# tiborcamargo/KinectPy

Hardware: AMD Instinct MI355X
Metric: Mpoints/sec end-to-end (unproject+filter+ICP), 4-sensor frame (higher is better)
Workload: dtype f64 decisions / f32 storage

## Files before the change

### kinectpy_amd/csrc/kpx_icp.hip

```cpp
#include <chrono>
#include <mutex>
#include <fcntl.h>
#include <memory>
#include <condition_variable>
#include <thread>
#include <atomic>
#include <sys/file.h>
#include <unistd.h>
#include <limits.h>
#include <stddef.h>
#include <string.h>
#include <stdio.h>
#include <time.h>
#include <stdlib.h>

#include "kpx_internal.h"
#include "kpx_linalg.h"
#include "kpx_fixed.h"

namespace kpx {

typedef double d4 __attribute__((ext_vector_type(4)));
#ifndef KPX_ICP_ACQ_FENCE
#define KPX_ICP_ACQ_FENCE 1
// ... 1023 lines not shown
    uint32_t my_cert = 0u;
    const bool certs = fuse.ticket && fuse.light_key && fuse.cert;
    if (PERSIST && k > 0) {
        if (lane < 16) {
            my_row = rowi[wave][lane][1];
#pragma unroll
            for (int a = 0; a < 3; ++a) { my_src[a] = rowsrc[wave][lane][a]; my_pt[a] = rowk[wave][lane][a]; my_nrm[a] = rowk[wave][lane][3 + a]; }
            my_prev = __float_as_int(rowk[wave][lane][6]);
            if (certs) my_cert = rowc[wave][lane];
        }
    } else if (lane < 16) {
        const int64_t r = row_base + lane < last ? row_base + lane : last;
        if (idx_cur || d2_cur) my_row = row_of[r];
#pragma unroll
        for (int a = 0; a < 3; ++a) my_src[a] = src_sorted[3 * r + a];
        if (PERSIST) {
#pragma unroll
            for (int a = 0; a < 3; ++a) rowsrc[wave][lane][a] = my_src[a];
            rowc[wave][lane] = 0u;
        }
        if (k > 0) {
            my_prev = idx_sorted[r];
#pragma unroll
            for (int a = 0; a < 3; ++a) my_pt[a] = ptgt_sorted[3 * r + a];
            if (certs) my_cert = fuse.cert[r];
        }
    }
    __shared__ double s_thist[kCertHist][12];
    if (PERSIST) {
        if (certs && k < kCertHist && tix < 12) s_thist[k][tix] = st->T[tix];
    } else if (certs && k > 0)
        for (int e = tix; e < 12 * (k < kCertHist ? k : kCertHist); e += kIThreads) (&s_thist[0][0])[e] = fuse.thist[e];
    GroupPre gpre;
    group_pre_load(gpre, group_box, n_groups, lane);
    if (!PERSIST && mode == 1 && k > 0 && lane < 16) {
        const float *np_ = tn + 3 * (int64_t)(my_prev > 0 ? my_prev : 0);
#pragma unroll
        for (int a = 0; a < 3; ++a) my_nrm[a] = np_[a];
    }
    const double *Tk = st->T;
    static_assert(sizeof(IcpState) % sizeof(double) == 0, "IcpState is copied as doubles");
    if (KPX_ICP_STATE_LDS && fuse.ticket && tix < sizeof(IcpState) / sizeof(double))
        reinterpret_cast<double *>(&s_state)[tix] = reinterpret_cast<const double *>(st)[tix];
    if (fuse.pair) {
        const IcpState *in = fuse.pair + ((k + 1) & 1);
        IcpState *out = fuse.pair + (k & 1);
        const unsigned long long *prev = fuse.ring + (int64_t)((k + 2) % 3) * kAccSet;
        if (k > 0 && tix < kAcc) s_sums[tix] = (int)tix < (mode == 1 ? kAcc : 17) ? fixed_total(prev, tix) : 0.0;
        if (tix == 0) s_state = *in;
        __syncthreads();
        if (s_state.done) {
            if (bid == 0 && tix == 0) *out = s_state;
            return;
        }
        __shared__ FinishScratch s_fs;
        if (k > 0 && wave == 0)
            icp_finish_wave(s_sums, n, mode, k - 1, fuse.max_iter, fuse.rel_fit, fuse.rel_rmse, &s_state, bid == 0 ? fuse.result : (double *)nullptr,
                            s_fs, lane);
        __syncthreads();
        if (bid == 0) {
            unsigned long long *next = fuse.ring + (int64_t)((k + 1) % 3) * kAccSet;
            for (int e = tix; e < kAccSet; e += kIThreads) next[e] = 0ull;
            if (tix == 0) {
                *out = s_state;
                if (k > 0 && fuse.progress)
                    __hip_atomic_store(fuse.progress, fuse.tag | ((unsigned long long)(s_state.done ? 1 : 0) << 32) | (unsigned long long)(unsigned)k,
                                       __ATOMIC_RELEASE, __HIP_MEMORY_SCOPE_SYSTEM);
            }
        }
        if (s_state.done) return;
        Tk = s_state.T;
        acc = fuse.ring + (int64_t)(k % 3) * kAccSet;
    } else if (st->done) return;
    bool skip = false;
    if (fuse.ticket && fuse.light_key) {
        const double key = PERSIST ? (k > 0 ? s_key : 0.0) : fuse.light_key[bid];
        skip = key > 0.0 && (st->motion + st->reach) * (1.0 + 1e-6) + 1e-6 < key;
    }
    __shared__ double s_light[kIWaves];
    const int nacc = mode == 1 ? kAcc : 17;
    if (tile_visits && tix == 0 && bid < kStampBlocks) { g_icp_stamp[bid][7] = skip ? 1ull : 0ull; g_icp_stamp[bid][6] = (unsigned long long)nblocks; }
    do {
    if (skip) break;
    __shared__ int32_t lists[kIWaves][kLScratch];
    __shared__ double rowd[kIWaves][16][kRowStride];
    __shared__ float rowf[kIWaves][16][kRowFStride];
    __shared__ double sh[kAcc][kIRows + 1];
    if (tile_visits && tix == 0 && bid < kStampBlocks) {
        g_icp_stamp[bid][0] = t_block_start;
        g_icp_stamp[bid][6] = (unsigned long long)nblocks;
    }
    phase_tick(tile_visits, 1, bid);
    if (certs && (k > 0 || PERSIST)) __syncthreads();
    if (PERSIST && fuse.stamp && tix == 0) {
        const unsigned long long t = wall_clock64();
        if (bid == 0) fuse.stamp[0] = t;
        atomicMax(&fuse.stamp[5], t);
        atomicMin(&fuse.stamp[10], t);
    }

    const double c_reach = certs ? st->reach : 0.0;
    double c_skin = 0.0;
    if (certs && k > 0) {
        const double lm = st->last_motion, md = sqrt(max_d2);
        if (lm <= (double)fuse.pol.calm * md) c_skin = fmin(fmax((double)fuse.pol.factor * lm, (double)fuse.pol.smin * md), (double)fuse.pol.smax * md);
    }
    bool my_active = true, my_certd = false;
    if (lane < 16) {
        const int64_t i = my_row;
        double s[3];
        xform_row(Tk, my_src, s);
        const double seed = row_seed(s);
        double bv = INFINITY;
        int32_t bj = INT_MAX;
        if (k > 0) {
            const int32_t p = my_prev;
            if (p >= 0) {
                const double tx = my_pt[0], ty = my_pt[1], tz = my_pt[2];
                const double t2 = fma(tx, tx, fma(ty, ty, tz * tz));
                double d = fma(s[0], -2.0 * tx, seed);
                d = fma(s[1], -2.0 * ty, d);
                d = fma(s[2], -2.0 * tz, d);
                bv = fma(1.0, t2, d);
                bj = p;
            }
        }
        const double clamp = (max_d2 + 1.0) * (1.0 + 9.31322574615478515625e-10) + ldexp(seed + t2max + 1.0, -38);
        if (!(bv <= clamp)) { bv = clamp; bj = INT_MAX; }
        double rb0 = bv - 1.0;
        if (certs) {
            double d1 = c_reach;
            if (bj != INT_MAX) {
                const double dx = s[0] - (double)my_pt[0], dy = s[1] - (double)my_pt[1], dz = s[2] - (double)my_pt[2];
                d1 = sqrt(fma(dz, dz, fma(dy, dy, dx * dx))) * (1.0 + 1e-12);
            }
            const bool keeps = (my_prev >= 0) == (bj != INT_MAX);
            const int kc = (int)(my_cert & 63u);
            const float Lc = __uint_as_float(my_cert & ~63u);
            double pc[3] = { 0.0, 0.0, 0.0 };
            if (Lc > 0.0f) {
                const double *Th = s_thist[kc];
                const double x = my_src[0], y = my_src[1], z = my_src[2];
#pragma unroll
                for (int a = 0; a < 3; ++a) pc[a] = fma(Th[4 * a], x, fma(Th[4 * a + 1], y, fma(Th[4 * a + 2], z, Th[4 * a + 3])));
            }
            const double ex = s[0] - pc[0], ey = s[1] - pc[1], ez = s[2] - pc[2];
            const double moved = sqrt(fma(ez, ez, fma(ey, ey, ex * ex))) * (1.0 + 1e-12);
            const bool certd = Lc > 0.0f && keeps && (d1 + moved) * (1.0 + 1e-6) + 1e-6 < (double)Lc;
            my_active = (!certd || fuse.cert_check) && row_base + lane <= last;
            my_certd = certd && row_base + lane <= last;
            if (certd && !fuse.cert_check) rb0 = -1.0;
            else if (c_skin > 0.0) { const double rr = d1 + c_skin; rb0 = fmax(rb0, rr * rr); }
        }
        rowd[wave][lane][0] = s[0]; rowd[wave][lane][1] = s[1]; rowd[wave][lane][2] = s[2];
        rowd[wave][lane][3] = rb0;
        rowd[wave][lane][4] = seed; rowd[wave][lane][5] = bv;
        rowi[wave][lane][0] = bj; rowi[wave][lane][1] = (int32_t)i;
#pragma unroll
        for (int a = 0; a < 3; ++a) { rowk[wave][lane][a] = my_pt[a]; rowk[wave][lane][3 + a] = my_nrm[a]; }
        rowk[wave][lane][6] = __int_as_float(my_prev);
    }
    if (PERSIST && fuse.stamp) {
        const bool searched = lane < 16 && my_active && !my_certd;
        const unsigned long long sm = __builtin_amdgcn_ballot_w64(searched);
        const unsigned long long np = __builtin_amdgcn_ballot_w64(searched && my_prev < 0);
        const unsigned long long nc = __builtin_amdgcn_ballot_w64(searched && (my_cert & ~63u) == 0u);
        if (lane == 0 && sm) {
            atomicAdd(&fuse.stamp[26], 1ull); atomicAdd(&fuse.stamp[27], (unsigned long long)__builtin_popcountll(sm));
            atomicAdd(&fuse.stamp[28], (unsigned long long)__builtin_popcountll(np)); atomicAdd(&fuse.stamp[29], (unsigned long long)__builtin_popcountll(nc));
        }
// ... 12 lines not shown
        w.best[r] = rowd[wave][rr][5];
        w.bcol[r] = rowi[wave][rr][0];
        w.rb0[r] = rowd[wave][rr][3];
    }
    w.skin = c_skin;
    w.act_mask = act_mask;
    w.light_gap2 = -1.0;
    w.dbg = (PERSIST && fuse.stamp && bid == 0 && wave == 0) ? fuse.stamp + 16 : (unsigned long long *)nullptr;
    phase_tick(tile_visits, 2, bid);
    if (PERSIST) chain_tick(fuse.stamp, 1, bid == 0 && tix == 0);
    const unsigned long long t_sweep = tile_visits ? wall_clock64() : 0ull;
    unsigned long long swept = 0ull;
    int lane_p = 0, wave_p = 0, q_p = 0, j_p = 0;
    int64_t row_base_p = 0;
    auto rederive = [&]() {
        lane_p = opaque_i((int)(threadIdx.x & 63)); wave_p = opaque_i((int)(threadIdx.x >> 6)); q_p = lane_p >> 4; j_p = lane_p & 15;
        row_base_p = ((int64_t)bid * kIWaves + wave_p) * kLRows;
    };
    if (act_mask != 0u) {
        wave_lds_fence();
        swept = sweep_wave<true, true, PERSIST>(w, Bs, orig, tile_box, group_box, n_groups, t2max, lists[wave], &gpre);
        rederive();
        if (certs && fuse.cert_check && j_p == 0) {
#pragma unroll
            for (int r = 0; r < 4; ++r) {
                const int rr = q_p + 4 * r;
                if (((certd_mask >> rr) & 1u) != 0u && w.bcol[r] != rowi[wave_p][rr][0]) {
                    if (atomicAdd(&g_cert_check[2], 1ull) == 0ull) {
                        g_cert_check[3] = (unsigned long long)k; g_cert_check[4] = (unsigned long long)(row_base_p + rr);
                        g_cert_check[5] = (unsigned long long)(unsigned)rowi[wave_p][rr][0]; g_cert_check[6] = (unsigned long long)(unsigned)w.bcol[r];
                        g_cert_check[7] = (unsigned long long)((PERSIST ? rowc[wave_p][rr] : fuse.cert[row_base_p + rr]) & ~63u);
                    }
                }
            }
        }
        if (certs && j_p == 0) {
#pragma unroll
            for (int r = 0; r < 4; ++r) {
                const int rr = q_p + 4 * r;
                if (((act_mask >> rr) & 1u) != 0u && ((certd_mask >> rr) & 1u) == 0u) {
                    typedef unsigned uu2 __attribute__((ext_vector_type(2)));
                    const uu2 pat = { 0u, w.sec[r] };
                    const double d2nd = w.sec[r] == 0xFFFFFFFFu ? INFINITY : __builtin_bit_cast(double, pat) - 1.0 - w.eps_out;
                    const double l2 = fmin(w.rb_out[r], d2nd);
                    const uint32_t lb = l2 > 0.0 && k < kCertHist ? (__float_as_uint(f32_down(sqrt(l2) * (1.0 - 1e-7))) & ~63u) : 0u;
                    const uint32_t cw = lb > 63u ? (lb | (uint32_t)k) : 0u;
                    if (PERSIST) rowc[wave_p][rr] = cw; else fuse.cert[row_base_p + rr] = cw;
                }
            }
        }
    }
    if (act_mask == 0u) rederive();
    __shared__ int s_cnt[kIWaves];
    if (lane_p == 0) s_cnt[wave_p] = __builtin_popcount(act_mask & ~certd_mask);
    const unsigned visited = (unsigned)(swept & 0xFFFFu);
    if (certs && fuse.cert_check && lane_p == 0) {
        if (bid == 0 && wave_p == 0 && g_cert_check[2] == 0ull) {
            g_cert_check[3] = (unsigned long long)k; g_cert_check[4] = __builtin_bit_cast(unsigned long long, st->last_motion);
            g_cert_check[5] = __builtin_bit_cast(unsigned long long, st->motion); g_cert_check[6] = __builtin_bit_cast(unsigned long long, c_skin);
        }
        atomicAdd(&g_cert_check[0], (unsigned long long)__builtin_popcount(certd_mask));
        atomicAdd(&g_cert_check[1], (unsigned long long)__builtin_popcount(act_mask & ~certd_mask));
    }
    if (lane_p == 0) s_light[wave_p] = act_mask == 0xFFFFu ? w.light_gap2 : -1.0;
    if (tile_visits && lane_p == 0 && bid < kStampBlocks && kIWaves <= 4) {
        unsigned long long *o = g_icp_wave[bid * 4 + wave_p];
        int with = 0;
#pragma unroll
        for (int r = 0; r < 4; ++r) with += (w.bcol[r] >= 0 && w.bcol[r] != INT_MAX) ? 1 : 0;
        o[0] = t_sweep; o[1] = wall_clock64(); o[2] = swept; o[3] = (unsigned long long)with;
    }
    phase_tick(tile_visits, 3, bid);
    if (PERSIST) chain_tick(fuse.stamp, 2, bid == 0 && lane_p == 0 && wave_p == 0);
    if (PERSIST && fuse.stamp && bid == 0 && lane_p == 0 && wave_p == 0) { fuse.stamp[13] = swept; fuse.stamp[14] = (unsigned long long)act_mask | ((unsigned long long)certd_mask << 16); }
    if (tile_visits && lane_p == 0) atomicAdd(tile_visits + ((bid * kIWaves + wave_p) & (kVisitSlots - 1)), (unsigned long long)visited);
    wave_lds_fence();
    if (j_p == 0) {
#pragma unroll
        for (int r = 0; r < 4; ++r) rowi[wave_p][q_p + 4 * r][0] = w.bcol[r];
    }
    wave_lds_fence();

    const int lane_e = lane_p, wave_e = wave_p;
    if (lane_e < 16) {
        const int col = wave_e * 16 + lane_e;
        for (int a = 0; a < nacc; ++a) sh[a][col] = 0.0;
        if (row_base_p + lane_e <= last) {
            const int32_t bj = rowi[wave_e][lane_e][0];
            const int64_t i = rowi[wave_e][lane_e][1];
            const bool none = bj < 0 || bj == INT_MAX;
            const int32_t out_j = none ? -1 : bj;
            const int32_t prev_j = __float_as_int(rowk[wave_e][lane_e][6]);
            const bool changed = k == 0 || out_j != prev_j;
            if (idx_cur) idx_cur[i] = out_j;
            if (PERSIST) rowk[wave_e][lane_e][6] = __int_as_float(out_j);
            else if (changed) idx_sorted[row_base_p + lane_e] = out_j;
            if (none) {
                if (d2_cur) d2_cur[i] = INFINITY;
            } else {
                const double s[3] = { rowd[wave_e][lane_e][0], rowd[wave_e][lane_e][1], rowd[wave_e][lane_e][2] };
                float tf[3] = { rowk[wave_e][lane_e][0], rowk[wave_e][lane_e][1], rowk[wave_e][lane_e][2] }, nf[3] = { rowk[wave_e][lane_e][3], rowk[wave_e][lane_e][4], rowk[wave_e][lane_e][5] };
                if (changed) {
                    const float *tp = tgt + 3 * (int64_t)bj;
#pragma unroll
                    for (int c = 0; c < 3; ++c) tf[c] = tp[c];
                    if (mode == 1) {
                        const float *np_ = tn + 3 * (int64_t)bj;
#pragma unroll
                        for (int c = 0; c < 3; ++c) nf[c] = np_[c];
                    }
#pragma unroll
                    for (int c = 0; c < 3; ++c) {
                        if (PERSIST) { rowk[wave_e][lane_e][c] = tf[c]; rowk[wave_e][lane_e][3 + c] = nf[c]; }
                        else ptgt_sorted[3 * (row_base_p + lane_e) + c] = tf[c];
                    }
                }
                const double t[3] = { (double)tf[0], (double)tf[1], (double)tf[2] };
                const double dx = s[0] - t[0], dy = s[1] - t[1], dz = s[2] - t[2];
                const double d2 = fma(dz, dz, fma(dy, dy, dx * dx));
                if (d2_cur) d2_cur[i] = d2;
                if (d2 < max_d2) {
                    sh[0][col] = 1.0; sh[1][col] = d2;
#pragma unroll
                    for (int c = 0; c < 3; ++c) { sh[2 + c][col] = s[c]; sh[5 + c][col] = t[c]; }
#pragma unroll
                    for (int a = 0; a < 3; ++a)
#pragma unroll
                        for (int c = 0; c < 3; ++c) sh[8 + 3 * a + c][col] = t[a] * s[c];
                    if (mode == 1) {
                        const double nx = nf[0], ny = nf[1], nz = nf[2];
                        const double res = (s[0] - t[0]) * nx + (s[1] - t[1]) * ny + (s[2] - t[2]) * nz;
                        const double J[6] = { s[1] * nz - s[2] * ny, s[2] * nx - s[0] * nz, s[0] * ny - s[1] * nx, nx, ny, nz };
                        int slot = 17;
#pragma unroll
                        for (int a = 0; a < 6; ++a)
#pragma unroll
                            for (int c = a; c < 6; ++c) sh[slot++][col] = J[a] * J[c];
#pragma unroll
                        for (int a = 0; a < 6; ++a) sh[38 + a][col] = J[a] * res;
                    }
                }
            }
        }
    }
    __syncthreads();
    phase_tick(tile_visits, 4, bid);
    const int tix_e = wave_e * 64 + lane_e;
    if (tix_e < nacc) {
        unsigned long long lo = 0ull, hi = 0ull;
#pragma unroll
        for (int t = 0; t < kIWaves; ++t) {
            unsigned long long l, h;
            fixed_split(tile_tree16(&sh[tix_e][16 * t]), l, h);
            fixed_accumulate(lo, hi, l, h);
        }
        unsigned long long *slot = acc + (((int64_t)(bid & (kAccCopies - 1)) * kAcc + tix_e) * kFixedWords);
        if (fuse.ticket) fixed_add_words_performed(slot, lo, hi); else fixed_add_words(slot, lo, hi);
    } else if (!PERSIST && fuse.ticket && tix_e == nacc) {
        int cnt = 0;
#pragma unroll
        for (int wv = 0; wv < kIWaves; ++wv) cnt += s_cnt[wv];
        if (cnt) {
            const unsigned long long back = __hip_atomic_fetch_add(fuse.ticket + kSearchedWord + (bid & 7u), (unsigned long long)cnt, __ATOMIC_RELAXED, __HIP_MEMORY_SCOPE_AGENT);
            asm volatile("" ::"v"(back));
        }
    }
    if (fuse.light_key && tix == kIThreads - 1) {
        double g2 = INFINITY;
        bool light = true;
#pragma unroll
        for (int wv = 0; wv < kIWaves; ++wv) { light = light && s_light[wv] >= 0.0; g2 = fmin(g2, s_light[wv]); }
        const double nk = light ? st->motion + sqrt(g2) * (1.0 - 1e-9) : 0.0;
        if (PERSIST) s_key = nk; else fuse.light_key[bid] = nk;
    }
    phase_tick(tile_visits, 5, bid);
    } while (false);
    if (PERSIST && fuse.stamp && tix == 0) {
        const unsigned long long t = wall_clock64();
        if (bid == 0) fuse.stamp[3] = t;
        atomicMax(&fuse.stamp[11], t);
    }
    if (!fuse.ticket) return;
    __shared__ unsigned s_ticket;
    __syncthreads();
    if (tix == 0) s_ticket = (unsigned)__hip_atomic_fetch_add(fuse.ticket, 1ull, __ATOMIC_RELAXED, __HIP_MEMORY_SCOPE_AGENT);
    __syncthreads();
    if (PERSIST && fuse.stamp && tix == 0) {
        const unsigned long long t = wall_clock64();
        if (bid == 0) fuse.stamp[4] = t;
        atomicMax(&fuse.stamp[6], t);
    }
    if (s_ticket != nblocks - 1u) return;
#if KPX_ICP_ACQ_FENCE
    __builtin_amdgcn_fence(__ATOMIC_ACQUIRE, "agent");
#endif
    const int tix_w = opaque_i((int)threadIdx.x);
    if (tix_w < kAcc) s_sums[tix_w] = tix_w < nacc ? fixed_total_coherent(acc, tix_w) : 0.0;
    const unsigned long long n_searched = PERSIST ? 0ull : searched_take(fuse.ticket, tix_w);
    __syncthreads();
    if (PERSIST) chain_tick(fuse.stamp, 7, tix == 0);
    for (int e = tix_w; e < kAccSet; e += kIThreads) __hip_atomic_store(acc + e, 0ull, __ATOMIC_RELAXED, __HIP_MEMORY_SCOPE_AGENT);
    if (tix == 0) __hip_atomic_store(fuse.ticket, 0ull, __ATOMIC_RELAXED, __HIP_MEMORY_SCOPE_AGENT);
    if (PERSIST) asm volatile("s_waitcnt vmcnt(0)" ::: "memory");
    if (wave != 0) {
        if (PERSIST) __syncthreads();
        return;
    }
    __shared__ FinishScratch s_tail;
    const double *tbbox_w = tbbox;
    asm volatile("" : "+s"(tbbox_w));
    const double t2max_w = target_t2max(tbbox_w);
    IcpState *stw = const_cast<IcpState *>(st);
    IcpState *work = KPX_ICP_STATE_LDS ? &s_state : stw;
    if (PERSIST)
        icp_finish_wave_call(s_sums, n, mode, k, fuse.max_iter, fuse.rel_fit, fuse.rel_rmse, work, (double *)nullptr, &s_tail, lane,
                             fuse.light_key ? fuse.sbbox : (const double *)nullptr, max_d2, t2max_w, fuse.stamp ? fuse.stamp + 32 : (unsigned long long *)nullptr);
    else
        icp_finish_wave(s_sums, n, mode, k, fuse.max_iter, fuse.rel_fit, fuse.rel_rmse, work, fuse.result, s_tail, lane,
                        LightSkip{ fuse.light_key ? fuse.sbbox : (const double *)nullptr, max_d2, t2max_w });
    wave_lds_fence();
    if (PERSIST) chain_tick(fuse.stamp, 8, lane == 0);
    if (PERSIST) {
        static_assert(KPX_ICP_STATE_LDS, "the chain form updates the LDS copy of the state");
        static_assert(sizeof(IcpState) == kChainWords * sizeof(double), "record layout");
        __syncthreads();
        if (lane < kChainWords)
            __hip_atomic_store(reinterpret_cast<unsigned long long *>(fuse.chain_rec + (size_t)kChainRec * (k + 1)) + lane,
                               reinterpret_cast<const unsigned long long *>(&s_state)[lane], __ATOMIC_RELAXED, __HIP_MEMORY_SCOPE_AGENT);
        if (work->done && fuse.result) {
            if (lane < 16) fuse.result[lane] = work->T[lane];
            if (lane == 0) { fuse.result[16] = work->fitness; fuse.result[17] = work->rmse; fuse.result[18] = (double)k; fuse.result[19] = work->count; }
        }
        if (lane == 0 && fuse.progress && work->done)
            __hip_atomic_store(fuse.progress, fuse.tag | (1ull << 32) | (unsigned long long)(unsigned)(k + 1), __ATOMIC_RELAXED, __HIP_MEMORY_SCOPE_SYSTEM);
        chain_tick(fuse.stamp, 9, lane == 0);
        if (fuse.stamp && lane == 0) fuse.stamp[12] = __builtin_amdgcn_s_memtime();
// ... 1532 lines not shown
```

### kinectpy_amd/csrc/kpx_icprows.h

```cpp
#pragma once

namespace kpx {

constexpr int kRowsBatchMax = 16;
constexpr int kRowsBlock = 64;
struct RowsProblem {
    const float *src_sorted;
    int32_t *idx_sorted;
    float *ptgt_sorted;
    uint32_t *cert;
    double *thist;
    double *light_key;
    const double *sbbox;
    IcpState *state;
    unsigned long long *ring;
    double *result;
    unsigned long long *progress;
    unsigned long long tag;
    const float *tgt, *tn;
    const double *Bs;
    const int32_t *orig;
    const float *tile_box, *group_box;
    const double *tbbox;
    int64_t n;
    int32_t n_groups, k;
    uint32_t block0, blocks;
};
struct RowsArgs {
    RowsProblem p[kRowsBatchMax];
    int32_t count;
};

constexpr int kDppXor1 = 0xB1, kDppXor2 = 0x4E, kDppHalfMirror = 0x141, kDppMirror = 0x140;
__device__ __forceinline__ double row16_tree_sum(double v)
{
    v += dpp_f64<kDppXor1>(v);
    v += dpp_f64<kDppXor2>(v);
    v += dpp_f64<kDppHalfMirror>(v);
    v += dpp_f64<kDppMirror>(v);
    return v;
}

template <int MODE, int R>
__global__ __launch_bounds__(64) __attribute__((amdgpu_waves_per_eu(KPX_ICP_WPE, KPX_ICP_WPE))) void icp_rows_kernel(RowsArgs args, double max_d2, int max_iter, double rel_fit,
                                                                                                                     double rel_rmse, unsigned long long *__restrict__ tile_visits,
                                                                                                                     int light, CertPolicy pol)
{
    constexpr int NACC = MODE == 1 ? kAcc : 17;
    static_assert(R == 16 || R == 32 || R == 64, "rows per wave");
    int pi = 0;
#pragma unroll
    for (int c = 1; c < kRowsBatchMax; ++c) pi += (c < args.count && blockIdx.x >= args.p[c].block0) ? 1 : 0;
    const RowsProblem &P = args.p[pi];
    const unsigned bid = blockIdx.x - P.block0;
    const int k = P.k;
    IcpState *const st = P.state;
    if (st->done) return;

    __shared__ IcpState s_state;
    __shared__ double s_sums[kAcc];
    __shared__ FinishScratch s_tail;
    __shared__ double rowd[kRowsBlock][kRowStride];
    __shared__ float rowf[kLRows][kRowFStride];
    __shared__ float rowk[kRowsBlock][11];
    __shared__ int32_t rowi[kRowsBlock];
    __shared__ uint32_t rowc[kRowsBlock];
    __shared__ int32_t rowm[kRowsBlock];
    __shared__ int32_t lists[kLScratch];
    static_assert(kLScratch * sizeof(int32_t) >= 4 * kAcc * sizeof(double), "the tile partials reuse the sweep's scratch");
    double (*s_part)[kAcc] = reinterpret_cast<double (*)[kAcc]>(lists);

    const int lane = threadIdx.x;
    const unsigned long long lt = (1ull << lane) - 1ull;
    const int64_t last = P.n - 1;
    const int64_t row = (int64_t)bid * R + lane;
    const bool valid = lane < R && row <= last;
    const int64_t r = valid ? row : last;
    const bool certs = (light & 2) != 0, use_light = (light & 1) != 0, cert_check = (light & 4) != 0;
    const double t2max = target_t2max(P.tbbox);

    float my_src[3], my_pt[3] = { 0.0f, 0.0f, 0.0f }, my_nrm[3] = { 0.0f, 0.0f, 0.0f };
    int32_t my_prev = -1;
    uint32_t my_cert = 0u;
#pragma unroll
    for (int a = 0; a < 3; ++a) my_src[a] = P.src_sorted[3 * r + a];
    if (k > 0) {
        my_prev = P.idx_sorted[r];
#pragma unroll
        for (int a = 0; a < 3; ++a) my_pt[a] = P.ptgt_sorted[3 * r + a];
        if (certs) my_cert = P.cert[r];
    }
    const double key_in = use_light ? P.light_key[bid] : 0.0;
    if (lane < (int)(sizeof(IcpState) / sizeof(double))) reinterpret_cast<double *>(&s_state)[lane] = reinterpret_cast<const double *>(st)[lane];
    GroupPre gpre;
    group_pre_load(gpre, P.group_box, P.n_groups, lane);
    if (MODE == 1 && k > 0) {
        const float *np_ = P.tn + 3 * (int64_t)(my_prev > 0 ? my_prev : 0);
#pragma unroll
        for (int a = 0; a < 3; ++a) my_nrm[a] = np_[a];
    }
    double Th[12];
    const int kc = (int)(my_cert & 63u);
    const float Lc = __uint_as_float(my_cert & ~63u);
    if (certs && k > 0 && Lc > 0.0f) {
#pragma unroll
        for (int e = 0; e < 12; ++e) Th[e] = P.thist[12 * kc + e];
    } else {
#pragma unroll
        for (int e = 0; e < 12; ++e) Th[e] = 0.0;
    }
    const double *Tk = st->T;
    unsigned long long *const ticket = P.ring + kAccSet;

    const bool skip = use_light && key_in > 0.0 && (st->motion + st->reach) * (1.0 + 1e-6) + 1e-6 < key_in;
    unsigned visited_total = 0u;
    if (!skip) {
        const double c_reach = certs ? st->reach : 0.0;
        double c_skin = 0.0;
        if (certs && k > 0) {
            const double lm = st->last_motion, md = sqrt(max_d2);
            if (lm <= (double)pol.calm * md) c_skin = fmin(fmax((double)pol.factor * lm, (double)pol.smin * md), (double)pol.smax * md);
        }
        bool my_active = valid, my_certd = false;
        unsigned long long act64, certd64;
        int n_act;
        {
            double s[3];
            xform_row(Tk, my_src, s);
            const double seed = row_seed(s);
            double bv = INFINITY;
            int32_t bj = INT_MAX;
            if (k > 0 && my_prev >= 0) {
                const double tx = my_pt[0], ty = my_pt[1], tz = my_pt[2];
                const double t2 = fma(tx, tx, fma(ty, ty, tz * tz));
                double d = fma(s[0], -2.0 * tx, seed);
                d = fma(s[1], -2.0 * ty, d);
                d = fma(s[2], -2.0 * tz, d);
                bv = fma(1.0, t2, d);
                bj = my_prev;
            }
            const double clamp = (max_d2 + 1.0) * (1.0 + 9.31322574615478515625e-10) + ldexp(seed + t2max + 1.0, -38);
            if (!(bv <= clamp)) { bv = clamp; bj = INT_MAX; }
            double rb0 = bv - 1.0;
            if (certs) {
                double d1 = c_reach;
                if (bj != INT_MAX) {
                    const double dx = s[0] - (double)my_pt[0], dy = s[1] - (double)my_pt[1], dz = s[2] - (double)my_pt[2];
                    d1 = sqrt(fma(dz, dz, fma(dy, dy, dx * dx))) * (1.0 + 1e-12);
                }
                const bool keeps = (my_prev >= 0) == (bj != INT_MAX);
                double pc[3] = { 0.0, 0.0, 0.0 };
                if (Lc > 0.0f) {
                    const double x = my_src[0], y = my_src[1], z = my_src[2];
#pragma unroll
                    for (int a = 0; a < 3; ++a) pc[a] = fma(Th[4 * a], x, fma(Th[4 * a + 1], y, fma(Th[4 * a + 2], z, Th[4 * a + 3])));
                }
                const double ex = s[0] - pc[0], ey = s[1] - pc[1], ez = s[2] - pc[2];
                const double moved = sqrt(fma(ez, ez, fma(ey, ey, ex * ex))) * (1.0 + 1e-12);
                const bool certd = Lc > 0.0f && keeps && (d1 + moved) * (1.0 + 1e-6) + 1e-6 < (double)Lc;
                my_active = (!certd || cert_check) && valid;
                my_certd = certd && valid;
                if (certd && !cert_check) rb0 = -1.0;
                else if (c_skin > 0.0) { const double rr = d1 + c_skin; rb0 = fmax(rb0, rr * rr); }
            }
            act64 = __builtin_amdgcn_ballot_w64(my_active);
            certd64 = __builtin_amdgcn_ballot_w64(my_certd);
            n_act = __builtin_popcountll(act64);
            if (my_active) {
                const int slot = __builtin_popcountll(act64 & lt);
                rowd[slot][0] = s[0]; rowd[slot][1] = s[1]; rowd[slot][2] = s[2];
                rowd[slot][3] = rb0;
                rowd[slot][4] = seed; rowd[slot][5] = bv;
                rowi[slot] = bj;
                rowc[slot] = my_cert;
                rowm[slot] = my_certd ? 1 : 0;
            }
            if (lane >= n_act) {
                rowd[lane][0] = 0.0; rowd[lane][1] = 0.0; rowd[lane][2] = 0.0;
                rowd[lane][3] = -1.0;
                rowd[lane][4] = 1.0; rowd[lane][5] = 2.0;
                rowi[lane] = INT_MAX;
                rowc[lane] = 0u;
                rowm[lane] = 1;
            }
#pragma unroll
            for (int a = 0; a < 3; ++a) { rowk[lane][a] = my_pt[a]; rowk[lane][3 + a] = my_nrm[a]; rowk[lane][7 + a] = my_src[a]; }
            rowk[lane][6] = __int_as_float(my_prev);
        }
        wave_lds_fence();

        bool light_blk = n_act == R;
        double gap2_blk = INFINITY;
#pragma unroll 1
        for (int v0 = 0; v0 < n_act; v0 += kLRows) {
            const int left = n_act - v0;
            const unsigned act_mask = left >= kLRows ? 0xFFFFu : ((1u << left) - 1u);
            const int lane_s = opaque_i((int)threadIdx.x), q_s = lane_s >> 4, j_s = lane_s & 15;
            WaveRows w;
            w.rows = &rowd[v0][0];
            w.rowsf = &rowf[0][0];
            w.a = q_s < 3 ? rowd[v0 + j_s][q_s] : 1.0;
#pragma unroll
            for (int rr4 = 0; rr4 < 4; ++rr4) {
                const int rr = v0 + q_s + 4 * rr4;
                w.seed[rr4] = rowd[rr][4];
                w.best[rr4] = rowd[rr][5];
                w.bcol[rr4] = rowi[rr];
                w.rb0[rr4] = rowd[rr][3];
            }
            w.skin = c_skin;
            w.act_mask = act_mask;
            w.light_gap2 = -1.0;
            w.dbg = nullptr;
            wave_lds_fence();
            const unsigned long long swept = sweep_wave<true, true, true>(w, P.Bs, P.orig, P.tile_box, P.group_box, P.n_groups, t2max, lists, &gpre);
            visited_total += (unsigned)(swept & 0xFFFFu);
            const int lane_p = opaque_i((int)threadIdx.x), q_p = lane_p >> 4, j_p = lane_p & 15;
            if (certs && cert_check && j_p == 0) {
#pragma unroll
                for (int rr4 = 0; rr4 < 4; ++rr4) {
                    const int rr = q_p + 4 * rr4;
                    if (((act_mask >> rr) & 1u) != 0u && rowm[v0 + rr] != 0 && w.bcol[rr4] != rowi[v0 + rr]) {
                        if (atomicAdd(&g_cert_check[2], 1ull) == 0ull) {
                            g_cert_check[3] = (unsigned long long)k; g_cert_check[4] = (unsigned long long)((int64_t)bid * R + v0 + rr);
                            g_cert_check[5] = (unsigned long long)(unsigned)rowi[v0 + rr]; g_cert_check[6] = (unsigned long long)(unsigned)w.bcol[rr4];
                            g_cert_check[7] = (unsigned long long)(rowc[v0 + rr] & ~63u);
                        }
                    }
                }
            }
            wave_lds_fence();
            if (j_p == 0) {
#pragma unroll
                for (int rr4 = 0; rr4 < 4; ++rr4) {
                    const int rr = q_p + 4 * rr4;
                    rowi[v0 + rr] = w.bcol[rr4];
                    if (certs && ((act_mask >> rr) & 1u) != 0u && rowm[v0 + rr] == 0) {
                        typedef unsigned uu2 __attribute__((ext_vector_type(2)));
                        const uu2 pat = { 0u, w.sec[rr4] };
                        const double d2nd = w.sec[rr4] == 0xFFFFFFFFu ? INFINITY : __builtin_bit_cast(double, pat) - 1.0 - w.eps_out;
                        const double l2 = fmin(w.rb_out[rr4], d2nd);
                        const uint32_t lb = l2 > 0.0 && k < kCertHist ? (__float_as_uint(f32_down(sqrt(l2) * (1.0 - 1e-7))) & ~63u) : 0u;
                        rowc[v0 + rr] = lb > 63u ? (lb | (uint32_t)k) : 0u;
                    }
                }
            }
            if (w.light_gap2 >= 0.0) gap2_blk = fmin(gap2_blk, w.light_gap2);
            else light_blk = false;
            wave_lds_fence();
        }
        const int lane_e = opaque_i((int)threadIdx.x);
        const unsigned long long lt_e = (1ull << lane_e) - 1ull;
        if (certs && cert_check && lane_e == 0) {
            if (bid == 0 && g_cert_check[2] == 0ull) {
                g_cert_check[3] = (unsigned long long)k; g_cert_check[4] = __builtin_bit_cast(unsigned long long, st->last_motion);
                g_cert_check[5] = __builtin_bit_cast(unsigned long long, st->motion); g_cert_check[6] = __builtin_bit_cast(unsigned long long, c_skin);
            }
            atomicAdd(&g_cert_check[0], (unsigned long long)__builtin_popcountll(certd64));
            atomicAdd(&g_cert_check[1], (unsigned long long)__builtin_popcountll(act64 & ~certd64));
        }
        if (tile_visits && lane_e == 0 && visited_total) atomicAdd(tile_visits + (blockIdx.x & (kVisitSlots - 1)), (unsigned long long)visited_total);

        double c[NACC];
#pragma unroll
        for (int a = 0; a < NACC; ++a) c[a] = 0.0;
        const int64_t row_e = (int64_t)bid * R + lane_e;
        if (lane_e < R && row_e <= last) {
            const bool was_act = ((act64 >> lane_e) & 1ull) != 0ull;
            const int slot_e = __builtin_popcountll(act64 & lt_e);
            const int32_t prev_j = __float_as_int(rowk[lane_e][6]);
            const int32_t bj = was_act ? rowi[slot_e] : (prev_j >= 0 ? prev_j : INT_MAX);
            const bool none = bj < 0 || bj == INT_MAX;
            const int32_t out_j = none ? -1 : bj;
            const bool changed = k == 0 || out_j != prev_j;
            if (changed) P.idx_sorted[row_e] = out_j;
            const bool searched = was_act && ((certd64 >> lane_e) & 1ull) == 0ull;
            if (certs && searched) P.cert[row_e] = rowc[slot_e];
            if (!none) {
                const float sf[3] = { rowk[lane_e][7], rowk[lane_e][8], rowk[lane_e][9] };
                double s[3];
                xform_row(Tk, sf, s);
                float tf[3] = { rowk[lane_e][0], rowk[lane_e][1], rowk[lane_e][2] }, nf[3] = { rowk[lane_e][3], rowk[lane_e][4], rowk[lane_e][5] };
                if (changed) {
                    const float *tp = P.tgt + 3 * (int64_t)bj;
#pragma unroll
                    for (int e = 0; e < 3; ++e) tf[e] = tp[e];
                    if (MODE == 1) {
                        const float *np_ = P.tn + 3 * (int64_t)bj;
#pragma unroll
                        for (int e = 0; e < 3; ++e) nf[e] = np_[e];
                    }
#pragma unroll
                    for (int e = 0; e < 3; ++e) P.ptgt_sorted[3 * row_e + e] = tf[e];
                }
                const double t[3] = { (double)tf[0], (double)tf[1], (double)tf[2] };
                const double dx = s[0] - t[0], dy = s[1] - t[1], dz = s[2] - t[2];
                const double d2 = fma(dz, dz, fma(dy, dy, dx * dx));
                if (d2 < max_d2) {
                    c[0] = 1.0; c[1] = d2;
#pragma unroll
                    for (int e = 0; e < 3; ++e) { c[2 + e] = s[e]; c[5 + e] = t[e]; }
#pragma unroll
                    for (int a = 0; a < 3; ++a)
#pragma unroll
                        for (int e = 0; e < 3; ++e) c[8 + 3 * a + e] = t[a] * s[e];
                    if (MODE == 1) {
                        const double nx = nf[0], ny = nf[1], nz = nf[2];
                        const double res = (s[0] - t[0]) * nx + (s[1] - t[1]) * ny + (s[2] - t[2]) * nz;
                        const double J[6] = { s[1] * nz - s[2] * ny, s[2] * nx - s[0] * nz, s[0] * ny - s[1] * nx, nx, ny, nz };
                        int slot = 17;
#pragma unroll
                        for (int a = 0; a < 6; ++a)
#pragma unroll
                            for (int e = a; e < 6; ++e) c[slot++] = J[a] * J[e];
#pragma unroll
                        for (int a = 0; a < 6; ++a) c[38 + a] = J[a] * res;
                    }
                }
            }
        }
#pragma unroll
        for (int a = 0; a < NACC; ++a) c[a] = row16_tree_sum(c[a]);
        wave_lds_fence();
        if ((lane_e & 15) == 0) {
#pragma unroll
            for (int a = 0; a < NACC; ++a) s_part[lane_e >> 4][a] = c[a];
        }
        wave_lds_fence();
        if (lane_e < NACC) {
            unsigned long long lo = 0ull, hi = 0ull;
#pragma unroll
            for (int t = 0; t < 4; ++t) {
                unsigned long long l, h;
                fixed_split(s_part[t][lane_e], l, h);
                fixed_accumulate(lo, hi, l, h);
            }
            fixed_add_words_performed(P.ring + (((int64_t)(bid & (kAccCopies - 1)) * kAcc + lane_e) * kFixedWords), lo, hi);
        } else if (lane_e == NACC && (act64 & ~certd64) != 0ull) {
            const unsigned long long back = __hip_atomic_fetch_add(ticket + kSearchedWord + (bid & 7u), (unsigned long long)__builtin_popcountll(act64 & ~certd64), __ATOMIC_RELAXED,
                                                                   __HIP_MEMORY_SCOPE_AGENT);
            asm volatile("" ::"v"(back));
        }
        if (use_light && lane_e == 0) P.light_key[bid] = light_blk ? st->motion + sqrt(gap2_blk) * (1.0 - 1e-9) : 0.0;
    }

    asm volatile("s_waitcnt vmcnt(0)" ::: "memory");
    unsigned tk = 0u;
    if (threadIdx.x == 0) tk = (unsigned)__hip_atomic_fetch_add(ticket, 1ull, __ATOMIC_RELAXED, __HIP_MEMORY_SCOPE_AGENT);
    tk = (unsigned)__builtin_amdgcn_readfirstlane((int)tk);
    if (tk != P.blocks - 1u) return;
#if KPX_ICP_ACQ_FENCE
    __builtin_amdgcn_fence(__ATOMIC_ACQUIRE, "agent");
#endif
    const int lane_w = opaque_i((int)threadIdx.x);
    if (lane_w < kAcc) s_sums[lane_w] = lane_w < NACC ? fixed_total_coherent(P.ring, lane_w) : 0.0;
    const unsigned long long n_searched = searched_take(ticket, lane_w);
    for (int e = lane_w; e < kAccSet; e += 64) __hip_atomic_store(P.ring + e, 0ull, __ATOMIC_RELAXED, __HIP_MEMORY_SCOPE_AGENT);
    if (lane_w == 0) __hip_atomic_store(ticket, 0ull, __ATOMIC_RELAXED, __HIP_MEMORY_SCOPE_AGENT);
    wave_lds_fence();
    const double *tbbox_w = P.tbbox;
    asm volatile("" : "+s"(tbbox_w));
    const double t2max_w = target_t2max(tbbox_w);
    icp_finish_wave(s_sums, P.n, MODE, k, max_iter, rel_fit, rel_rmse, &s_state, P.result, s_tail, lane_w,
                    LightSkip{ use_light ? P.sbbox : (const double *)nullptr, max_d2, t2max_w });
    wave_lds_fence();
    if (lane_w < (int)(sizeof(IcpState) / sizeof(double))) reinterpret_cast<double *>(st)[lane_w] = reinterpret_cast<const double *>(&s_state)[lane_w];
    if (certs && k + 1 < kCertHist && lane_w < 12) P.thist[12 * (k + 1) + lane_w] = s_state.T[lane_w];
    if (lane_w == 0 && P.progress)
        __hip_atomic_store(P.progress, P.tag | progress_searched(n_searched, P.n) | ((unsigned long long)(s_state.done ? 1 : 0) << 32) | (unsigned long long)(unsigned)(k + 1),
                           __ATOMIC_RELAXED, __HIP_MEMORY_SCOPE_SYSTEM);
}

}
```

### kinectpy_amd/csrc/kpx_nnlocal.h

```cpp
#pragma once
#include "kpx_morton.h"

namespace kpx {

constexpr int kLGroupTiles = 16;
constexpr int kLRows = 16;
constexpr int kLList = 320;
constexpr int kVisitSlots = 1024;

__global__ __launch_bounds__(256) void nn_local_prep_kernel(const float *__restrict__ tgt, int64_t m, double *__restrict__ Bs,
                                                            int32_t *__restrict__ orig, float *__restrict__ tile_box,
                                                            float *__restrict__ group_box)
{
    const int64_t j = (int64_t)blockIdx.x * 256 + threadIdx.x;
    double b0 = 0.0, b1 = 0.0, b2 = 0.0, b3 = kSentinel;
    float lo[3] = { kBoxBig, kBoxBig, kBoxBig }, hi[3] = { -kBoxBig, -kBoxBig, -kBoxBig };
    if (j < m) {
        const int64_t o = orig[j];
        const float fx = tgt[3 * o], fy = tgt[3 * o + 1], fz = tgt[3 * o + 2];
        const double tx = fx, ty = fy, tz = fz;
        b0 = -2.0 * tx; b1 = -2.0 * ty; b2 = -2.0 * tz;
        b3 = fma(tx, tx, fma(ty, ty, tz * tz));
        lo[0] = hi[0] = fx; lo[1] = hi[1] = fy; lo[2] = hi[2] = fz;
    } else {
// ... 7 lines not shown
        for (int msk = 1; msk < 16; msk <<= 1) {
            lo[a] = fminf(lo[a], __shfl_xor(lo[a], msk, 64));
            hi[a] = fmaxf(hi[a], __shfl_xor(hi[a], msk, 64));
        }
    __shared__ float sb[16][6];
    if ((threadIdx.x & 15) == 0) {
        float *tb = tile_box + (j >> 4) * 6;
#pragma unroll
        for (int a = 0; a < 3; ++a) { tb[a] = lo[a]; tb[3 + a] = hi[a]; sb[threadIdx.x >> 4][a] = lo[a]; sb[threadIdx.x >> 4][3 + a] = hi[a]; }
    }
    __syncthreads();
    if (threadIdx.x < 6) {
        float v = sb[0][threadIdx.x];
        for (int t = 1; t < 16; ++t) v = threadIdx.x < 3 ? fminf(v, sb[t][threadIdx.x]) : fmaxf(v, sb[t][threadIdx.x]);
        group_box[(int64_t)blockIdx.x * 6 + threadIdx.x] = v;
    }
}

__global__ __launch_bounds__(256) void nn_local_rowprep_kernel(const float *__restrict__ src, int64_t n, const float *__restrict__ tgt,
                                                               const double *__restrict__ T, const int32_t *__restrict__ done,
                                                               const int32_t *__restrict__ row_of, const int32_t *__restrict__ prev,
                                                               double max_d2, const double *__restrict__ tbbox,
                                                               double *__restrict__ init_val, int32_t *__restrict__ init_idx,
                                                               double *__restrict__ A64, double *__restrict__ K64)
{
    if (done && *done) return;
    const int64_t r = (int64_t)blockIdx.x * blockDim.x + threadIdx.x;
    if (r >= n) return;
    const int64_t i = row_of[r];
    double s[3];
    xform_row(T, src + 3 * i, s);
    const double seed = row_seed(s);
    reinterpret_cast<double2 *>(A64)[2 * r] = make_double2(s[0], s[1]);
    reinterpret_cast<double2 *>(A64)[2 * r + 1] = make_double2(s[2], 1.0);
    K64[r] = seed;
    double bv = INFINITY;
    int32_t bj = INT_MAX;
    if (prev) {
        const int32_t j = prev[i];
        if (j >= 0 && j != INT_MAX) {
            const float *tp = tgt + 3 * (int64_t)j;
            const double tx = tp[0], ty = tp[1], tz = tp[2];
            const double t2 = fma(tx, tx, fma(ty, ty, tz * tz));
            double d = fma(s[0], -2.0 * tx, seed);
            d = fma(s[1], -2.0 * ty, d);
            d = fma(s[2], -2.0 * tz, d);
            bv = fma(1.0, t2, d);
            bj = j;
        }
    }
    if (max_d2 > 0.0) {
        double t2max = 0.0;
#pragma unroll
        for (int a = 0; a < 3; ++a) t2max += fmax(tbbox[a] * tbbox[a], tbbox[3 + a] * tbbox[3 + a]);
        const double clamp = (max_d2 + 1.0) * (1.0 + 9.31322574615478515625e-10) + ldexp(seed + t2max + 1.0, -38);
        if (!(bv <= clamp)) { bv = clamp; bj = INT_MAX; }
    }
    init_val[r] = bv;
    init_idx[r] = bj;
}

__device__ __forceinline__ unsigned fold16(unsigned long long m) { return (unsigned)((m | (m >> 16) | (m >> 32) | (m >> 48)) & 0xFFFFull); }

template <int CTRL>
__device__ __forceinline__ int dpp_i32(int v) { return __builtin_amdgcn_update_dpp(v, v, CTRL, 0xF, 0xF, false); }
template <int CTRL>
__device__ __forceinline__ double dpp_f64(double v)
{
    typedef int i2 __attribute__((ext_vector_type(2)));
    i2 b = __builtin_bit_cast(i2, v);
    b[0] = dpp_i32<CTRL>(b[0]);
    b[1] = dpp_i32<CTRL>(b[1]);
    return __builtin_bit_cast(double, b);
}
constexpr int kRor1 = 0x121, kRor2 = 0x122, kRor4 = 0x124, kRor8 = 0x128;
__device__ __forceinline__ double row16_all_max(double v)
{
    v = fmax(v, dpp_f64<kRor1>(v)); v = fmax(v, dpp_f64<kRor2>(v)); v = fmax(v, dpp_f64<kRor4>(v)); v = fmax(v, dpp_f64<kRor8>(v));
    return v;
}
__device__ __forceinline__ double row16_all_min(double v)
{
    v = fmin(v, dpp_f64<kRor1>(v)); v = fmin(v, dpp_f64<kRor2>(v)); v = fmin(v, dpp_f64<kRor4>(v)); v = fmin(v, dpp_f64<kRor8>(v));
    return v;
}
__device__ __forceinline__ double readlane_f64(double v, int l)
{
    typedef int i2 __attribute__((ext_vector_type(2)));
    i2 b = __builtin_bit_cast(i2, v);
    b[0] = __builtin_amdgcn_readlane(b[0], l);
    b[1] = __builtin_amdgcn_readlane(b[1], l);
    return __builtin_bit_cast(double, b);
}
__device__ __forceinline__ double wave_uniform_max(double v)
{
    v = row16_all_max(v);
    return fmax(fmax(readlane_f64(v, 0), readlane_f64(v, 16)), fmax(readlane_f64(v, 32), readlane_f64(v, 48)));
}

__device__ __forceinline__ double quad_uniform_max(double v)
{
    return fmax(fmax(readlane_f64(v, 0), readlane_f64(v, 16)), fmax(readlane_f64(v, 32), readlane_f64(v, 48)));
}

__device__ __forceinline__ float f32_down(double x)
{
    float f = (float)x;
    if ((double)f > x) f = f > 0.0f ? __int_as_float(__float_as_int(f) - 1) : (f < 0.0f ? __int_as_float(__float_as_int(f) + 1) : -1.401298464e-45f);
    return f;
}
__device__ __forceinline__ float f32_up(double x)
{
    float f = (float)x;
    if ((double)f < x) f = f > 0.0f ? __int_as_float(__float_as_int(f) + 1) : (f < 0.0f ? __int_as_float(__float_as_int(f) - 1) : 1.401298464e-45f);
    return f;
}
__device__ __forceinline__ float pt_gap2_lb(const float *__restrict__ pf, const float lo[3], const float hi[3])
{
    const float gx = fmaxf(0.0f, fmaxf(lo[0] - pf[3], pf[0] - hi[0]));
    const float gy = fmaxf(0.0f, fmaxf(lo[1] - pf[4], pf[1] - hi[1]));
    const float gz = fmaxf(0.0f, fmaxf(lo[2] - pf[5], pf[2] - hi[2]));
    return fmaf(gz, gz, fmaf(gy, gy, gx * gx)) * 0.99999904632568359375f;
}

struct WaveRows {
    double a;
    d4 seed;
    double *rows;
    float *rowsf;
    double best[4];
    int32_t bcol[4];
    double light_gap2;
    double rb0[4];
    double skin;
    unsigned act_mask;
    unsigned sec[4];
    double rb_out[4], eps_out;
    unsigned long long *dbg;
};
constexpr int kRowStride = 6, kRowBound = 3;
constexpr int kRowFStride = 8, kRowFBound = 6;

constexpr int kLCand = 16, kLSurv = 16;
constexpr int kLScratch = kLList + 7 * kLCand + 2 * kLSurv;
#ifndef KPX_MUL_BATCH
#define KPX_MUL_BATCH 8
#endif
constexpr int kMulBatch = KPX_MUL_BATCH;
#ifndef KPX_TIGHTEN_GAIN
#define KPX_TIGHTEN_GAIN 0.5
#endif
constexpr double kTightenGain = KPX_TIGHTEN_GAIN;

constexpr int kGroupPre = 2;
struct GroupPre {
    float b[kGroupPre][6];
};
__device__ __forceinline__ void group_box_load(float b[6], const float *__restrict__ group_box, int32_t n_groups, int gi)
{
    const bool on = gi < n_groups;
    const float *bx = group_box + (int64_t)(on ? gi : 0) * 6;
#pragma unroll
    for (int a = 0; a < 3; ++a) { b[a] = on ? bx[a] : kBoxBig; b[3 + a] = on ? bx[3 + a] : -kBoxBig; }
}
__device__ __forceinline__ void group_pre_load(GroupPre &g, const float *__restrict__ group_box, int32_t n_groups, int lane)
{
// ... 375 lines not shown
```

Baseline: 2470.

## Reduce ICP tile partials in registers via DPP and reuse sweep scratch LDS

The per-row accumulator epilogue in the ICP tile kernel no longer writes every accumulator term into a large shared array that a 16-wide tree then reads back. All 64 lanes now compute each row's terms and split them into quarters, one quarter per lane group. Each quarter is reduced across the 16 rows with DPP row sums, and the per-wave partials go into the sweep's list scratch, which lets the sh shared array be removed. This cuts LDS footprint and traffic and may raise occupancy, at the cost of duplicated per-lane arithmetic and more register pressure. The rows kernel also moves its gap2 minimum into LDS, recomputes t2max from tbbox inside the loop, and fuses the DPP sum with the partial store.

After: 2503 (median of 6 runs). +1.3%, better.

```diff
diff --git a/kinectpy_amd/csrc/kpx_icp.hip b/kinectpy_amd/csrc/kpx_icp.hip
--- a/kinectpy_amd/csrc/kpx_icp.hip
+++ b/kinectpy_amd/csrc/kpx_icp.hip
@@ -1129,10 +1129,9 @@
     if (tile_visits && tix == 0 && bid < kStampBlocks) { g_icp_stamp[bid][7] = skip ? 1ull : 0ull; g_icp_stamp[bid][6] = (unsigned long long)nblocks; }
     do {
     if (skip) break;
-    __shared__ int32_t lists[kIWaves][kLScratch];
+    __shared__ __attribute__((aligned(16))) int32_t lists[kIWaves][kLScratch];
     __shared__ double rowd[kIWaves][16][kRowStride];
     __shared__ float rowf[kIWaves][16][kRowFStride];
-    __shared__ double sh[kAcc][kIRows + 1];
     if (tile_visits && tix == 0 && bid < kStampBlocks) {
         g_icp_stamp[bid][0] = t_block_start;
         g_icp_stamp[bid][6] = (unsigned long long)nblocks;
@@ -1311,65 +1310,92 @@
     wave_lds_fence();
 
     const int lane_e = lane_p, wave_e = wave_p;
-    if (lane_e < 16) {
-        const int col = wave_e * 16 + lane_e;
-        for (int a = 0; a < nacc; ++a) sh[a][col] = 0.0;
-        if (row_base_p + lane_e <= last) {
-            const int32_t bj = rowi[wave_e][lane_e][0];
-            const int64_t i = rowi[wave_e][lane_e][1];
-            const bool none = bj < 0 || bj == INT_MAX;
-            const int32_t out_j = none ? -1 : bj;
-            const int32_t prev_j = __float_as_int(rowk[wave_e][lane_e][6]);
-            const bool changed = k == 0 || out_j != prev_j;
-            if (idx_cur) idx_cur[i] = out_j;
-            if (PERSIST) rowk[wave_e][lane_e][6] = __int_as_float(out_j);
-            else if (changed) idx_sorted[row_base_p + lane_e] = out_j;
-            if (none) {
-                if (d2_cur) d2_cur[i] = INFINITY;
-            } else {
-                const double s[3] = { rowd[wave_e][lane_e][0], rowd[wave_e][lane_e][1], rowd[wave_e][lane_e][2] };
-                float tf[3] = { rowk[wave_e][lane_e][0], rowk[wave_e][lane_e][1], rowk[wave_e][lane_e][2] }, nf[3] = { rowk[wave_e][lane_e][3], rowk[wave_e][lane_e][4], rowk[wave_e][lane_e][5] };
-                if (changed) {
-                    const float *tp = tgt + 3 * (int64_t)bj;
-#pragma unroll
-                    for (int c = 0; c < 3; ++c) tf[c] = tp[c];
-                    if (mode == 1) {
-                        const float *np_ = tn + 3 * (int64_t)bj;
-#pragma unroll
-                        for (int c = 0; c < 3; ++c) nf[c] = np_[c];
-                    }
-#pragma unroll
-                    for (int c = 0; c < 3; ++c) {
-                        if (PERSIST) { rowk[wave_e][lane_e][c] = tf[c]; rowk[wave_e][lane_e][3 + c] = nf[c]; }
-                        else ptgt_sorted[3 * (row_base_p + lane_e) + c] = tf[c];
-                    }
+    if (lane_e < 16 && row_base_p + lane_e <= last) {
+        const int32_t bj = rowi[wave_e][lane_e][0];
+        const int64_t i = rowi[wave_e][lane_e][1];
+        const bool none = bj < 0 || bj == INT_MAX;
+        const int32_t out_j = none ? -1 : bj;
+        const int32_t prev_j = __float_as_int(rowk[wave_e][lane_e][6]);
+        const bool changed = k == 0 || out_j != prev_j;
+        if (idx_cur) idx_cur[i] = out_j;
+        if (PERSIST) rowk[wave_e][lane_e][6] = __int_as_float(out_j);
+        else if (changed) idx_sorted[row_base_p + lane_e] = out_j;
+        if (none) {
+            if (d2_cur) d2_cur[i] = INFINITY;
+        } else if (changed) {
+            float tf[3], nf[3] = { rowk[wave_e][lane_e][3], rowk[wave_e][lane_e][4], rowk[wave_e][lane_e][5] };
+            const float *tp = tgt + 3 * (int64_t)bj;
+#pragma unroll
+            for (int c = 0; c < 3; ++c) tf[c] = tp[c];
+            if (mode == 1) {
+                const float *np_ = tn + 3 * (int64_t)bj;
+#pragma unroll
+                for (int c = 0; c < 3; ++c) nf[c] = np_[c];
+            }
+#pragma unroll
+            for (int c = 0; c < 3; ++c) {
+                rowk[wave_e][lane_e][c] = tf[c]; rowk[wave_e][lane_e][3 + c] = nf[c];
+                if (!PERSIST) ptgt_sorted[3 * (row_base_p + lane_e) + c] = tf[c];
+            }
+        }
+        if (!none && d2_cur) {
+            const double dx = rowd[wave_e][lane_e][0] - (double)rowk[wave_e][lane_e][0], dy = rowd[wave_e][lane_e][1] - (double)rowk[wave_e][lane_e][1],
+                         dz = rowd[wave_e][lane_e][2] - (double)rowk[wave_e][lane_e][2];
+            d2_cur[i] = fma(dz, dz, fma(dy, dy, dx * dx));
+        }
+    }
+    wave_lds_fence();
+    constexpr int kQuarter = (kAcc + 3) / 4;
+    static_assert(kLScratch * sizeof(int32_t) >= kAcc * sizeof(double), "the tile partials reuse the sweep's scratch");
+    {
+        const int q_e = lane_e >> 4, j_e = lane_e & 15;
+        double c[kQuarter];
+#pragma unroll
+        for (int e = 0; e < kQuarter; ++e) c[e] = 0.0;
+        const int32_t bj = rowi[wave_e][j_e][0];
+        if (row_base_p + j_e <= last && bj >= 0 && bj != INT_MAX) {
+            const double s[3] = { rowd[wave_e][j_e][0], rowd[wave_e][j_e][1], rowd[wave_e][j_e][2] };
+            const double t[3] = { (double)rowk[wave_e][j_e][0], (double)rowk[wave_e][j_e][1], (double)rowk[wave_e][j_e][2] };
+            const double dx = s[0] - t[0], dy = s[1] - t[1], dz = s[2] - t[2];
+            const double d2 = fma(dz, dz, fma(dy, dy, dx * dx));
+            if (d2 < max_d2) {
+                double v[4 * kQuarter];
+                v[0] = 1.0; v[1] = d2;
+#pragma unroll
+                for (int e = 0; e < 3; ++e) { v[2 + e] = s[e]; v[5 + e] = t[e]; }
+#pragma unroll
+                for (int a = 0; a < 3; ++a)
+#pragma unroll
+                    for (int e = 0; e < 3; ++e) v[8 + 3 * a + e] = t[a] * s[e];
+#pragma unroll
+                for (int e = 17; e < 4 * kQuarter; ++e) v[e] = 0.0;
+                if (mode == 1) {
+                    const double nx = rowk[wave_e][j_e][3], ny = rowk[wave_e][j_e][4], nz = rowk[wave_e][j_e][5];
+                    const double res = (s[0] - t[0]) * nx + (s[1] - t[1]) * ny + (s[2] - t[2]) * nz;
+                    const double J[6] = { s[1] * nz - s[2] * ny, s[2] * nx - s[0] * nz, s[0] * ny - s[1] * nx, nx, ny, nz };
+                    int slot = 17;
+#pragma unroll
+                    for (int a = 0; a < 6; ++a)
+#pragma unroll
+                        for (int e = a; e < 6; ++e) v[slot++] = J[a] * J[e];
+#pragma unroll
+                    for (int a = 0; a < 6; ++a) v[38 + a] = J[a] * res;
                 }
-                const double t[3] = { (double)tf[0], (double)tf[1], (double)tf[2] };
-                const double dx = s[0] - t[0], dy = s[1] - t[1], dz = s[2] - t[2];
-                const double d2 = fma(dz, dz, fma(dy, dy, dx * dx));
-                if (d2_cur) d2_cur[i] = d2;
-                if (d2 < max_d2) {
-                    sh[0][col] = 1.0; sh[1][col] = d2;
-#pragma unroll
-                    for (int c = 0; c < 3; ++c) { sh[2 + c][col] = s[c]; sh[5 + c][col] = t[c]; }
-#pragma unroll
-                    for (int a = 0; a < 3; ++a)
-#pragma unroll
-                        for (int c = 0; c < 3; ++c) sh[8 + 3 * a + c][col] = t[a] * s[c];
-                    if (mode == 1) {
-                        const double nx = nf[0], ny = nf[1], nz = nf[2];
-                        const double res = (s[0] - t[0]) * nx + (s[1] - t[1]) * ny + (s[2] - t[2]) * nz;
-                        const double J[6] = { s[1] * nz - s[2] * ny, s[2] * nx - s[0] * nz, s[0] * ny - s[1] * nx, nx, ny, nz };
-                        int slot = 17;
-#pragma unroll
-                        for (int a = 0; a < 6; ++a)
-#pragma unroll
-                            for (int c = a; c < 6; ++c) sh[slot++][col] = J[a] * J[c];
-#pragma unroll
-                        for (int a = 0; a < 6; ++a) sh[38 + a][col] = J[a] * res;
-                    }
+#pragma unroll
+                for (int e = 0; e < kQuarter; ++e) {
+                    double x0 = v[e], x1 = v[kQuarter + e], x2 = v[2 * kQuarter + e], x3 = v[3 * kQuarter + e];
+                    asm("" : "+v"(x0), "+v"(x1), "+v"(x2), "+v"(x3));
+                    c[e] = q_e == 0 ? x0 : q_e == 1 ? x1 : q_e == 2 ? x2 : x3;
                 }
             }
+        }
+#pragma unroll
+        for (int e = 0; e < kQuarter; ++e) c[e] = row16_tree_sum(c[e]);
+        double *part = reinterpret_cast<double *>(lists[wave_e]);
+        if (j_e == 0) {
+#pragma unroll
+            for (int e = 0; e < kQuarter; ++e)
+                if (kQuarter * q_e + e < kAcc) part[kQuarter * q_e + e] = c[e];
         }
     }
     __syncthreads();
@@ -1380,7 +1406,7 @@
 #pragma unroll
         for (int t = 0; t < kIWaves; ++t) {
             unsigned long long l, h;
-            fixed_split(tile_tree16(&sh[tix_e][16 * t]), l, h);
+            fixed_split(reinterpret_cast<const double *>(lists[t])[tix_e], l, h);
             fixed_accumulate(lo, hi, l, h);
         }
         unsigned long long *slot = acc + (((int64_t)(bid & (kAccCopies - 1)) * kAcc + tix_e) * kFixedWords);
diff --git a/kinectpy_amd/csrc/kpx_icprows.h b/kinectpy_amd/csrc/kpx_icprows.h
--- a/kinectpy_amd/csrc/kpx_icprows.h
+++ b/kinectpy_amd/csrc/kpx_icprows.h
@@ -31,16 +31,6 @@
     int32_t count;
 };
 
-constexpr int kDppXor1 = 0xB1, kDppXor2 = 0x4E, kDppHalfMirror = 0x141, kDppMirror = 0x140;
-__device__ __forceinline__ double row16_tree_sum(double v)
-{
-    v += dpp_f64<kDppXor1>(v);
-    v += dpp_f64<kDppXor2>(v);
-    v += dpp_f64<kDppHalfMirror>(v);
-    v += dpp_f64<kDppMirror>(v);
-    return v;
-}
-
 template <int MODE, int R>
 __global__ __launch_bounds__(64) __attribute__((amdgpu_waves_per_eu(KPX_ICP_WPE, KPX_ICP_WPE))) void icp_rows_kernel(RowsArgs args, double max_d2, int max_iter, double rel_fit,
                                                                                                                      double rel_rmse, unsigned long long *__restrict__ tile_visits,
@@ -59,6 +49,7 @@
 
     __shared__ IcpState s_state;
     __shared__ double s_sums[kAcc];
+    __shared__ double s_gap2;
     __shared__ FinishScratch s_tail;
     __shared__ double rowd[kRowsBlock][kRowStride];
     __shared__ float rowf[kLRows][kRowFStride];
@@ -186,11 +177,11 @@
 #pragma unroll
             for (int a = 0; a < 3; ++a) { rowk[lane][a] = my_pt[a]; rowk[lane][3 + a] = my_nrm[a]; rowk[lane][7 + a] = my_src[a]; }
             rowk[lane][6] = __int_as_float(my_prev);
+            if (lane == 0) s_gap2 = INFINITY;
         }
         wave_lds_fence();
 
         bool light_blk = n_act == R;
-        double gap2_blk = INFINITY;
 #pragma unroll 1
         for (int v0 = 0; v0 < n_act; v0 += kLRows) {
             const int left = n_act - v0;
@@ -213,7 +204,9 @@
             w.light_gap2 = -1.0;
             w.dbg = nullptr;
             wave_lds_fence();
-            const unsigned long long swept = sweep_wave<true, true, true>(w, P.Bs, P.orig, P.tile_box, P.group_box, P.n_groups, t2max, lists, &gpre);
+            const double *tbbox_s = P.tbbox;
+            asm volatile("" : "+s"(tbbox_s));
+            const unsigned long long swept = sweep_wave<true, true, true>(w, P.Bs, P.orig, P.tile_box, P.group_box, P.n_groups, target_t2max(tbbox_s), lists, &gpre);
             visited_total += (unsigned)(swept & 0xFFFFu);
             const int lane_p = opaque_i((int)threadIdx.x), q_p = lane_p >> 4, j_p = lane_p & 15;
             if (certs && cert_check && j_p == 0) {
@@ -245,7 +238,7 @@
                     }
                 }
             }
-            if (w.light_gap2 >= 0.0) gap2_blk = fmin(gap2_blk, w.light_gap2);
+            if (w.light_gap2 >= 0.0) { if (j_p == 0 && q_p == 0) s_gap2 = fmin(s_gap2, w.light_gap2); }
             else light_blk = false;
             wave_lds_fence();
         }
@@ -320,11 +313,9 @@
             }
         }
 #pragma unroll
-        for (int a = 0; a < NACC; ++a) c[a] = row16_tree_sum(c[a]);
-        wave_lds_fence();
-        if ((lane_e & 15) == 0) {
-#pragma unroll
-            for (int a = 0; a < NACC; ++a) s_part[lane_e >> 4][a] = c[a];
+        for (int a = 0; a < NACC; ++a) {
+            const double v = row16_tree_sum(c[a]);
+            if ((lane_e & 15) == 0) s_part[lane_e >> 4][a] = v;
         }
         wave_lds_fence();
         if (lane_e < NACC) {
@@ -341,7 +332,7 @@
                                                                    __HIP_MEMORY_SCOPE_AGENT);
             asm volatile("" ::"v"(back));
         }
-        if (use_light && lane_e == 0) P.light_key[bid] = light_blk ? st->motion + sqrt(gap2_blk) * (1.0 - 1e-9) : 0.0;
+        if (use_light && lane_e == 0) P.light_key[bid] = light_blk ? st->motion + sqrt(s_gap2) * (1.0 - 1e-9) : 0.0;
     }
 
     asm volatile("s_waitcnt vmcnt(0)" ::: "memory");
diff --git a/kinectpy_amd/csrc/kpx_nnlocal.h b/kinectpy_amd/csrc/kpx_nnlocal.h
--- a/kinectpy_amd/csrc/kpx_nnlocal.h
+++ b/kinectpy_amd/csrc/kpx_nnlocal.h
@@ -113,6 +113,15 @@
 __device__ __forceinline__ double row16_all_min(double v)
 {
     v = fmin(v, dpp_f64<kRor1>(v)); v = fmin(v, dpp_f64<kRor2>(v)); v = fmin(v, dpp_f64<kRor4>(v)); v = fmin(v, dpp_f64<kRor8>(v));
+    return v;
+}
+constexpr int kDppXor1 = 0xB1, kDppXor2 = 0x4E, kDppHalfMirror = 0x141, kDppMirror = 0x140;
+__device__ __forceinline__ double row16_tree_sum(double v)
+{
+    v += dpp_f64<kDppXor1>(v);
+    v += dpp_f64<kDppXor2>(v);
+    v += dpp_f64<kDppHalfMirror>(v);
+    v += dpp_f64<kDppMirror>(v);
     return v;
 }
 __device__ __forceinline__ double readlane_f64(double v, int l)
```
